# KMASAHIRO/AVR

Hardware: AMD Instinct MI355X
Metric: ray-samples/sec/GPU (1024 rays×256 samp×512 freq) + IR render ms/pose (higher is better)
Workload: dtype f32; 1 GPU; c2_meshrir_1024x256x512; mode=pose, rays=1024, samples=256, T=1022, freq_bins=512, distinct_poses=16, parallelism=poses x1 (no data-path collective)

## Files before the change

avr_amd/_lib.py:

```python
from __future__ import annotations

import ctypes
import math
import os
import threading

import numpy as np

_HERE = os.path.dirname(os.path.abspath(__file__))
LIB_PATH = os.path.join(_HERE, "libavr_hip.so")

DTYPE_F32 = 0
DTYPE_F16 = 1
DTYPE_BF16 = 2
MAX_AZI = 512

_c_i32 = ctypes.c_int32
_c_i64 = ctypes.c_int64
_c_f32 = ctypes.c_float
_vp = ctypes.c_void_p


class RenderParams(ctypes.Structure):

# ... 35 lines not shown
    p.n_samples = int(cfg["n_samples"])
    p.T = int(T)
    p.n_rays = p.n_azi * p.n_ele + 2 if n_rays is None else int(n_rays)
    p.depth_scale = _f32(cfg["far"] - cfg["near"])
    p.depth_offset = _f32(cfg["near"])
    p.lo = _f32(cfg["xyz_min"])
    p.span = _f32(cfg["xyz_max"] - cfg["xyz_min"])
    p.fs = _f32(cfg["fs"])
    p.speed = _f32(cfg["speed"])
    p.pathloss = _f32(cfg["pathloss"])
    p.azi_jitter = _f32(np.pi * 2 / cfg["n_azi"])
    p.two_pi = _f32(np.pi * 2)
    p.phase_c = _f32((-2 * np.pi) / T)
    p.near_clamp = int(0.1 / cfg["speed"] * cfg["fs"])
    p.pl_len = int(math.ceil(T * 2.5))
    return p


class TablePtrs(ctypes.Structure):

    _fields_ = [("d_vals", ctypes.c_void_p), ("shift", ctypes.c_void_p),
                ("pl_table", ctypes.c_void_p), ("phase", ctypes.c_void_p),
                ("twiddle", ctypes.c_void_p), ("ir_twiddle", ctypes.c_void_p)]


_SIGS = {
    "avr_last_error": (ctypes.c_char_p, []),
    "avr_abi_version": (ctypes.c_int, []),
    "avr_pinned_alloc": (ctypes.c_int, [_c_i64, _vp, _vp]),
    "avr_pinned_free": (ctypes.c_int, [_vp]),
    "avr_graph_launch": (ctypes.c_int, [_vp, _vp]),
    "avr_tables": (ctypes.c_int, [_vp, _vp, _vp, _vp, _vp, _vp, _vp, _vp]),
    "avr_depth_samples": (ctypes.c_int, [_vp, _vp, _vp]),
    "avr_ir_twiddle": (ctypes.c_int, [_c_i32, _vp, _vp]),
    "avr_ray_directions": (ctypes.c_int, [_vp, _vp, _vp, _vp]),
    "avr_sample_points": (ctypes.c_int, [_vp, _c_i32] + [_vp] * 10),
    "avr_sample_rays": (ctypes.c_int, [_vp, _c_i32, _vp, _c_i32] + [_vp] * 9),
    "avr_weights_fwd": (ctypes.c_int, [_vp, _c_i32, _vp, _c_i32] + [_vp] * 7),
    "avr_ray_reduce_fwd": (ctypes.c_int, [_vp, _c_i32, _vp, _c_i32, _vp, _vp, _c_i32, _vp, _vp]),
    "avr_sample_rays_dev": (ctypes.c_int, [_vp, _c_i32, _vp, _c_i32] + [_vp] * 9),
    "avr_sample_rays_staged": (ctypes.c_int, [_vp, _c_i32, _vp, _c_i32, _c_i32] + [_vp] * 7),
    "avr_reduce_splits": (ctypes.c_int, [_vp, _c_i32, _c_i32, _vp]),
    "avr_dft_phase_fwd": (ctypes.c_int, [_vp, _c_i32, _vp, _c_i32, _vp, _vp, _vp, _vp, _c_i32, _vp, _vp]),
    "avr_spectrum_finalize": (ctypes.c_int, [_c_i32, _c_i32, _c_i32, _vp, _vp, _vp]),
    "avr_irfft": (ctypes.c_int, [_c_i32, _c_i32, _vp, _vp, _vp, _vp]),
    "avr_irfft_bwd": (ctypes.c_int, [_c_i32, _c_i32, _vp, _vp, _vp, _vp]),
# ... 35 lines not shown
    "avr_head_bwd2": (ctypes.c_int, [_vp, _c_i32, _c_i32, _vp, _vp, _c_i32, _vp, _vp, _vp, _vp, _vp, _vp,
                                     _c_i32, _vp, _vp, _vp, _vp, _c_i64, _vp]),
    "avr_criterion_window_len": (ctypes.c_int, []),
    "avr_criterion_workspace": (ctypes.c_int, [_c_i32, _c_i32, _vp]),
    "avr_criterion_fwd": (ctypes.c_int, [_c_i32, _c_i32] + [_vp] * 10 + [_c_i64, _vp]),
    "avr_criterion_fwd2": (ctypes.c_int, [_c_i32, _c_i32] + [_vp] * 11 + [_c_i64, _vp]),
    "avr_criterion_bwd": (ctypes.c_int, [_c_i32, _c_i32] + [_vp] * 11 + [_c_i64, _vp, _vp]),
    "avr_das_workspace": (ctypes.c_int, [_vp]),
    "avr_das_fwd": (ctypes.c_int, [_c_i32] + [_vp] * 5 + [_c_f32] * 3 + [_vp, _vp, _c_i64, _vp]),
    "avr_das_bwd": (ctypes.c_int, [_c_i32] + [_vp] * 3 + [_c_f32] * 3 + [_vp, _vp, _c_i64, _vp, _vp]),
    "avr_scale_sanitize": (ctypes.c_int, [_c_i32, _vp, _vp, _vp, _vp]),
    "avr_grad_clip_workspace": (ctypes.c_int, [_c_i32, _vp, _vp]),
    "avr_grad_clip_coef": (ctypes.c_int, [_c_i32, _vp, _vp, ctypes.c_float, _vp, ctypes.c_int64, _vp, _vp, _vp]),
    "avr_adam_step": (ctypes.c_int, [_c_i32, _vp, _vp, _vp, _vp, _vp, _vp, _vp, ctypes.c_double, ctypes.c_double,
                                     ctypes.c_float, ctypes.c_float, _vp, _vp]),
    "avr_concat_fwd": (ctypes.c_int, [_c_i64, _c_i32, _vp, _vp, _c_i32, _vp]),
    "avr_concat_bwd": (ctypes.c_int, [_c_i64, _c_i32, _vp, _vp, _c_i32, _vp, _vp]),
    "avr_sigma_pack_bytes": (ctypes.c_int, [_c_i32, _vp]),
    "avr_sigma_desc_size": (ctypes.c_int, []),
    "avr_sigma_fwd": (ctypes.c_int, [_vp] * 3 + [_c_i32, _vp, _vp]),
    "avr_render_core_layout": (ctypes.c_int, [_vp, _c_i32, _c_i32, _vp, _vp]),
    "avr_render_core_fwd": (ctypes.c_int, [_vp, _c_i32, _vp, _c_i32, _vp, _c_i32] + [_vp] * 5
                            + [_c_i64] + [_vp] * 5),
}

EXPORTS = tuple(_SIGS)

_SHAPES_SIGS = {
    "avr_linear512_pack_w": (ctypes.c_int, [_vp, _c_i32, _vp, _vp]),
    "avr_linear512_relu_fwd": (ctypes.c_int, [_c_i64, _vp, _vp, _c_i32, _vp, _vp]),
    "avr_mlp512x2_pack_w": (ctypes.c_int, [_vp, _vp, _c_i32, _vp, _vp]),
    "avr_mlp512x2_fwd": (ctypes.c_int, [_c_i64, _vp, _vp, _c_i32, _vp, _vp]),
    "avr_linear_pack_w": (ctypes.c_int, [_c_i32, _c_i32, _vp, _c_i32, _vp, _vp]),
}

_lock = threading.Lock()
_lib = None


def load():
    global _lib
    if _lib is not None:
        return _lib
    with _lock:
        if _lib is not None:
            return _lib
# ... 27 lines not shown
```

avr_amd/csrc/common.h:

```cpp
#pragma once

#include <hip/hip_runtime.h>
#include <hip/hip_fp16.h>
#include <hip/hip_bf16.h>
#include <type_traits>
#include <stdint.h>
#include <string>

#include "avr_hip.h"

namespace avr {

void set_error(const std::string& msg);
int fail(int code, const std::string& msg);
int check_launch(const char* what);
int device_cus();

#define AVR_REQUIRE(cond, msg)                          \
    do {                                                \
        if (!(cond)) return ::avr::fail(AVR_E_ARG, msg); \
    } while (0)

int launch_irfft(int B, int F, const float* spec, const float* spec2, const float* tw, float* ir,
                 float* ir2, void* stream);

inline hipStream_t as_stream(void* s) { return reinterpret_cast<hipStream_t>(s); }

__device__ __forceinline__ void mfma_queue_wait() {
    __builtin_amdgcn_sched_barrier(0);
    asm volatile("s_nop 7");
}
template <typename T>
__device__ __forceinline__ void keep_live(const T& v) {
    asm volatile("" ::"v"(v));
}

__device__ __forceinline__ float load_f(const float* p, int64_t i) { return p[i]; }
__device__ __forceinline__ float load_f(const __half* p, int64_t i) { return __half2float(p[i]); }
__device__ __forceinline__ float load_f(const __hip_bfloat16* p, int64_t i) {
    return __bfloat162float(p[i]);
}
__device__ __forceinline__ void store_f(float* p, int64_t i, float v) { p[i] = v; }
__device__ __forceinline__ void store_f(__half* p, int64_t i, float v) { p[i] = __float2half(v); }
__device__ __forceinline__ void store_f(__hip_bfloat16* p, int64_t i, float v) {
    p[i] = __float2bfloat16(v);
}
__device__ __forceinline__ float bf16_lo(uint32_t u) { return __uint_as_float(u << 16); }
// ... 174 lines not shown
```

avr_amd/csrc/render_fwd.hip:

```cpp
#include "common.h"

#include <cstdlib>

using namespace avr;

typedef float floatx16 __attribute__((ext_vector_type(16)));

namespace {

constexpr double kTwoPi = 6.283185307179586476925286766559;

__global__ void tables_kernel(avr_render_params p, float* __restrict__ d_vals,
                              float* __restrict__ frac, int32_t* __restrict__ shift,
                              float* __restrict__ pl, float2* __restrict__ phase,
                              float2* __restrict__ tw) {
    const int S = p.n_samples, T = p.T, F = T / 2 + 1;
    const int64_t gid = (int64_t)blockIdx.x * blockDim.x + threadIdx.x;
    const int64_t stride = (int64_t)gridDim.x * blockDim.x;
    for (int64_t i = gid; i < S; i += stride) {
        const float d = linspace_at(0.0f, 1.0f, S, (int)i) * p.depth_scale + p.depth_offset;
        const float fr = (p.fs * d) / p.speed;
        d_vals[i] = d;
        frac[i] = fr;
        shift[i] = (int32_t)rintf(fr);
// ... 1019 lines not shown
    avr_reduce_splits(p, B, sig_dtype, &ns);
    L.n_split = ns;
    const int nkc = (int)((T + kKc - 1) / kKc);
    int ks = 1;
    if (const char* f = getenv("AVR_KSPLIT")) {
        ks = atoi(f);
    } else {
        const int64_t base = ((F + 127) / 128) * ((S + 31) / 32) * B;
        ks = (int)((256 + (base > 0 ? base : 1) - 1) / (base > 0 ? base : 1));
    }
    if (ks < 1) ks = 1;
    if (ks > nkc) ks = nkc;
    L.k_split = ks;
    L.P = (int32_t)(((S + 31) / 32) * ks);
    auto al = [](int64_t x) { return (x + 255) & ~(int64_t)255; };
    int64_t o = 0;
    L.w = o;
    o += al((int64_t)B * R * S * 4);
    L.delay = o;
    o += al((int64_t)B * R * S * 4);
    L.part = o;
    o += al((int64_t)ns * B * S * T * 4);
    L.spart = o;
    o += al((int64_t)B * L.P * F * 8);
    L.bytes = o;
    return L;
}
}

extern "C" int avr_render_core_layout(const avr_render_params* p, int32_t B, int32_t sig_dtype,
                                      int64_t* offsets ,
                                      int32_t* splits ) {
    if (int e = validate(p)) return e;
    AVR_REQUIRE(B >= 1 && offsets && splits, "avr_render_core_layout: bad args");
    const CoreLayout L = core_layout(p, B, sig_dtype);
    offsets[0] = L.w;
    offsets[1] = L.delay;
    offsets[2] = L.part;
    offsets[3] = L.spart;
    offsets[4] = L.bytes;
    splits[0] = L.n_split;
    splits[1] = L.k_split;
    return 0;
}

extern "C" int avr_render_core_fwd(const avr_render_params* p, int32_t B, const void* attn,
                                   int32_t attn_dtype, const void* signal, int32_t sig_dtype,
                                   const float* rays_o, const float* pos_tx, const float* dirs,
                                   const avr_table_ptrs* tab, void* workspace,
                                   int64_t workspace_bytes, float* out, float* ir, void* ev_begin,
                                   void* ev_end, void* stream) {
    if (int e = validate(p)) return e;
    AVR_REQUIRE(tab && workspace && out, "avr_render_core_fwd: null pointer");
    const CoreLayout L = core_layout(p, B, sig_dtype);
    AVR_REQUIRE(workspace_bytes >= L.bytes, "avr_render_core_fwd: workspace too small");
    char* ws = reinterpret_cast<char*>(workspace);
    float* w = reinterpret_cast<float*>(ws + L.w);
    int32_t* delay = reinterpret_cast<int32_t*>(ws + L.delay);
    float* part = reinterpret_cast<float*>(ws + L.part);
    float* spart = reinterpret_cast<float*>(ws + L.spart);
    if (int e = avr_weights_fwd(p, B, attn, attn_dtype, rays_o, pos_tx, dirs, tab->d_vals, w, delay, stream))
        return e;
    hipStream_t s = as_stream(stream);
    if (ev_begin) (void)hipEventRecord(reinterpret_cast<hipEvent_t>(ev_begin), s);
    if (int e = avr_ray_reduce_fwd(p, B, signal, sig_dtype, w, delay, L.n_split, part, stream))
        return e;
    if (ev_end) (void)hipEventRecord(reinterpret_cast<hipEvent_t>(ev_end), s);
    if (int e = avr_dft_phase_fwd(p, B, part, L.n_split, tab->pl_table, tab->shift, tab->phase, tab->twiddle,
                                  L.k_split, spart, stream))
        return e;
    if (int e = avr_spectrum_finalize(B, L.P, p->T / 2 + 1, spart, out, stream)) return e;
    if (ir) {
        AVR_REQUIRE(tab->ir_twiddle, "avr_render_core_fwd: ir requested without ir_twiddle");
        return avr_irfft(B, p->T / 2 + 1, out, tab->ir_twiddle, ir, stream);
    }
    return 0;
}
```

avr_amd/renderer.py:

```python
from __future__ import annotations

import ctypes
import math
import threading

import torch
import torch.nn as nn

from . import _lib
from ._lib import DTYPE_BF16, DTYPE_F16, DTYPE_F32, render_params
from .options import tuning_env
from .wcache import cache_lookup, cache_store, capturing, cast_weight


_RENDER_KEYS = ("n_samples", "near", "far", "n_azi", "n_ele", "speed", "fs", "pathloss",
                "xyz_min", "xyz_max")


def _ptr(t):
    return None if t is None else t.data_ptr()


def _stream(device):
    return torch.cuda.current_stream(device).cuda_stream
# ... 38 lines not shown
        f32 = dict(dtype=torch.float32, device=device)
        self.d_vals = torch.empty(S, **f32)
        self.frac = torch.empty(S, **f32)
        self.shift = torch.empty(S, dtype=torch.int32, device=device)
        self.pl = torch.empty(p.pl_len, **f32)
        self.phase = torch.empty(S, F, 2, **f32)
        self.twiddle = torch.empty(T, 2, **f32)
        n = 2 * (F - 1)
        self.ir_n = n
        self.ir_twiddle = torch.empty(max(n, 2), 2, **f32)
        st = _stream(device)
        with torch.cuda.device(device):
            _lib.call("avr_tables", ctypes_ref(p), _ptr(self.d_vals), _ptr(self.frac),
                      _ptr(self.shift), _ptr(self.pl), _ptr(self.phase), _ptr(self.twiddle), st)
            if n >= 2:
                _lib.call("avr_ir_twiddle", n, _ptr(self.ir_twiddle), st)
        shifts = self.shift.cpu()
        self.max_shift = int(shifts.max().item()) if S > 0 else 0
        self.ptrs = _lib.TablePtrs(self.d_vals.data_ptr(), self.shift.data_ptr(),
                                   self.pl.data_ptr(), self.phase.data_ptr(),
                                   self.twiddle.data_ptr(),
                                   self.ir_twiddle.data_ptr() if n >= 2 else None)
        self._layouts = {}

    def core_layout(self, p, B, sig_code):
        key = (p.n_rays, B, sig_code) + tuning_env()
        v = self._layouts.get(key)
        if v is None:
            with _TABLE_LOCK:
                v = self._layouts.get(key)
                if v is None:
                    off = (ctypes.c_int64 * 5)()
                    sp = (ctypes.c_int32 * 2)()
                    _lib.call("avr_render_core_layout", ctypes_ref(p), B, sig_code, off, sp)
                    v = (tuple(off), int(sp[0]), int(sp[1]))
                    self._layouts[key] = v
        return v


def ctypes_ref(p):
    import ctypes

    return ctypes.byref(p)


_TABLE_CACHE: dict = {}
# ... 33 lines not shown

def pick_k_split(B, S, T):
    F = T // 2 + 1
    nkc = math.ceil(T / 64)
    forced = tuning_env()[1]
    forced = int(forced) if forced else None
    if forced:
        return max(1, min(nkc, forced))
    base = math.ceil(F / 128) * math.ceil(S / 32) * B
    return max(1, min(nkc, math.ceil(256 / max(1, base))))


def _weights(p, attn, rays_o, position_tx, dirs, tables, st):
    B = attn.size(0)
    R, S = p.n_rays, p.n_samples
    dev = attn.device
    w = torch.empty(B, R, S, dtype=torch.float32, device=dev)
    delay = torch.empty(B, R, S, dtype=torch.int32, device=dev)
    _lib.call("avr_weights_fwd", ctypes_ref(p), B, _ptr(attn), _dtype_code(attn), _ptr(rays_o),
              _ptr(position_tx), _ptr(dirs), _ptr(tables.d_vals), _ptr(w), _ptr(delay), st)
    return w, delay


def _spectrum(p, tables, part, n_split, B, dev, st):
    S, T = p.n_samples, p.T
    F = T // 2 + 1
    k_split = pick_k_split(B, S, T)
    P = math.ceil(S / 32) * k_split
    spart = torch.empty(B, P, F, 2, dtype=torch.float32, device=dev)
    _lib.call("avr_dft_phase_fwd", ctypes_ref(p), B, _ptr(part), n_split, _ptr(tables.pl),
              _ptr(tables.shift), _ptr(tables.phase), _ptr(tables.twiddle), k_split,
              _ptr(spart), st)
    out = torch.empty(B, F, 2, dtype=torch.float32, device=dev)
    _lib.call("avr_spectrum_finalize", B, P, F, _ptr(spart), _ptr(out), st)
    return out


def _grad_z(p, tables, grad_out, B, dev, st):
    g = grad_out.contiguous().float()
    gz = torch.empty(B, p.n_samples, p.T, dtype=torch.float32, device=dev)
    _lib.call("avr_dft_phase_bwd", ctypes_ref(p), B, _ptr(g), _ptr(tables.pl), _ptr(tables.shift),
              _ptr(tables.phase), _ptr(tables.twiddle), _ptr(gz), st)
    return gz


def _grad_attn(p, tables, attn, grad_w, st):
    grad_attn = torch.empty_like(attn)
    _lib.call("avr_weights_bwd", ctypes_ref(p), attn.size(0), _ptr(attn), _dtype_code(attn),
              _ptr(tables.d_vals), _ptr(grad_w), _ptr(grad_attn), st)
    return grad_attn


def _render_core_fwd(attn, signal, p, tables, rays_o, position_tx, dirs, ir_out, timer=None):
    dev = signal.device
    B = signal.size(0)
    F = p.T // 2 + 1
    sig_code = _dtype_code(signal)
    off, n_split, _ = tables.core_layout(p, B, sig_code)
    ws = torch.empty(off[4], dtype=torch.uint8, device=dev)
    out = torch.empty(B, F, 2, dtype=torch.float32, device=dev)
    ev0 = ev1 = None
    if timer is not None:
        R, S = p.n_rays, p.n_samples
        delay = ws[off[1]:off[1] + B * R * S * 4].view(torch.int32).view(B, R, S)
        ev0, ev1 = timer.events(n_split=n_split, delay=delay, shift=tables.shift)
    _lib.call("avr_render_core_fwd", ctypes_ref(p), B, _ptr(attn), _dtype_code(attn),
              _ptr(signal), sig_code, _ptr(rays_o), _ptr(position_tx), _ptr(dirs),
              ctypes.byref(tables.ptrs), _ptr(ws), off[4], _ptr(out), _ptr(ir_out), ev0, ev1,
              _stream(dev))
    return out, ws, off


class RenderCore(torch.autograd.Function):

    @staticmethod
    def forward(ctx, attn, signal, p, tables, rays_o, position_tx, dirs, ir_out=None, timer=None):
        out, ws, off = _render_core_fwd(attn, signal, p, tables, rays_o, position_tx, dirs, ir_out, timer)
        B, R, S = signal.size(0), p.n_rays, p.n_samples
        w = ws[off[0]:off[0] + B * R * S * 4].view(torch.float32).view(B, R, S)
        delay = ws[off[1]:off[1] + B * R * S * 4].view(torch.int32).view(B, R, S)
        ctx.p, ctx.tables = p, tables
        ctx.save_for_backward(attn, signal, w, delay)
        return out

    @staticmethod
    def backward(ctx, grad_out):
        attn, signal, w, delay = ctx.saved_tensors
        p, tables = ctx.p, ctx.tables
        dev = signal.device
        B = signal.size(0)
        R, S = p.n_rays, p.n_samples
        st = _stream(dev)
        gz = _grad_z(p, tables, grad_out, B, dev, st)
        grad_signal = torch.empty_like(signal)
        grad_w = torch.empty(B, R, S, dtype=torch.float32, device=dev)
        _lib.call("avr_ray_reduce_bwd", ctypes_ref(p), B, _ptr(signal), _dtype_code(signal),
                  _ptr(gz), _ptr(w), _ptr(delay), _ptr(grad_signal), _ptr(grad_w), st)
        grad_attn = _grad_attn(p, tables, attn, grad_w, st) if ctx.needs_input_grad[0] else None
        return (grad_attn, grad_signal if ctx.needs_input_grad[1] else None,
                None, None, None, None, None, None, None)


def _packed_head_weight(w_master, W, cache, pref, shape_key, st):
    key = (W.data_ptr(), w_master._version, shape_key)
    cache = cache and not capturing()
    if cache:
        hit = cache_lookup(w_master, "_avr_headpack", key)
        if hit is not None:
            return hit
    B, K, code = shape_key[2], shape_key[3], shape_key[4]
    Wp = torch.empty_like(W)
    _lib.call("avr_head_pack_w", pref, B, K, _ptr(W), code, _ptr(Wp), st)
    return cache_store(w_master, "_avr_headpack", key, Wp) if cache else Wp


def _packed_exact_weight(w_master, W, cache, pref, shape_key, nbytes, st):
    key = (W.data_ptr(), w_master._version, shape_key)
    cache = cache and not capturing()
    if cache:
        hit = cache_lookup(w_master, "_avr_exactpack", key)
        if hit is not None:
            return hit
    K, code = shape_key[1], shape_key[2]
    Wf = torch.empty(nbytes // 2, dtype=W.dtype, device=W.device)
    _lib.call("avr_head_pack_w_exact", pref, K, _ptr(W), code, _ptr(Wf), st)
    return cache_store(w_master, "_avr_exactpack", key, Wf) if cache else Wf


class FusedHeadCore(torch.autograd.Function):

    @staticmethod
    def forward(ctx, attn, h, w_master, dtype, p, tables, rays_o, position_tx, dirs, cache=False, exact=False,
                relu_h=False, timer=None):
        dev = h.device
        B, K = h.size(0), h.size(-1)
        S, T = p.n_samples, p.T
        st = _stream(dev)
        pref = ctypes_ref(p)
        W = cast_weight(w_master, dtype, cache)
        code = _dtype_code(h)
        w, delay = _weights(p, attn, rays_o, position_tx, dirs, tables, st)
        R = p.n_rays
        perm = torch.empty(B, S, R, dtype=torch.int32, device=dev)
        ws = torch.empty(B, S, R, dtype=torch.float32, device=dev)
        cnt = torch.empty(B, S, T, dtype=torch.int32, device=dev)
        _lib.call("avr_head_sort", pref, B, _ptr(w), _ptr(delay), _ptr(perm), _ptr(ws), _ptr(cnt), st)
        if exact:
            ns, wbytes = ctypes.c_int32(0), ctypes.c_int64(0)
            _lib.call("avr_head_exact_layout", pref, B, K, code, ctypes.byref(ns), ctypes.byref(wbytes))
            n_split = ns.value
            part = torch.empty(n_split, B, S, T, dtype=torch.float32, device=dev)
            queue = torch.empty(256, dtype=torch.int32, device=dev)
            Wf = _packed_exact_weight(w_master, W, cache, pref, (p.T, K, code), wbytes.value, st)
            ev0, ev1 = timer.head_events(delay, tables.shift, K) if timer is not None else (None, None)
            if ev0 is not None:
                ev0.record()
            _lib.call("avr_head_fwd_exact", pref, B, K, _ptr(h), _ptr(Wf), code, _ptr(perm), _ptr(ws), _ptr(cnt),
                      _ptr(delay), n_split, _ptr(part), _ptr(queue), st)
            if ev1 is not None:
                ev1.record()
        else:
            ns = ctypes.c_int32(0)
            _lib.call("avr_head_splits", pref, B, K, code, ctypes.byref(ns))
            n_split = ns.value
            part = torch.empty(n_split, B, S, T, dtype=torch.float32, device=dev)
            Wp = _packed_head_weight(w_master, W, cache, pref, (p.T, R, B, K, code), st)
            _lib.call("avr_head_fwd", pref, B, K, _ptr(h), _ptr(Wp), code, _ptr(perm), _ptr(ws), _ptr(cnt),
                      n_split, _ptr(part), st)
        out = _spectrum(p, tables, part, n_split, B, dev, st)
        ctx.p, ctx.tables, ctx.relu_h = p, tables, relu_h
        ctx.save_for_backward(attn, h, W, w, delay, perm, ws, cnt)
        return out

    @staticmethod
    def backward(ctx, grad_out):
        attn, h, W, w, delay, perm, ws, cnt = ctx.saved_tensors
        p, tables = ctx.p, ctx.tables
        dev = h.device
        B, K = h.size(0), h.size(-1)
        R, S, T = p.n_rays, p.n_samples, p.T
        st = _stream(dev)
        pref = ctypes_ref(p)
        code = _dtype_code(h)
        gz = _grad_z(p, tables, grad_out, B, dev, st)
        nbytes = ctypes.c_int64(0)
        _lib.call("avr_head_bwd_workspace", pref, B, K, code, ctypes.byref(nbytes))
        work = torch.empty(max(1, nbytes.value // 4), dtype=torch.float32, device=dev)
        grad_h = torch.empty_like(h)
        grad_w = torch.empty(B, R, S, dtype=torch.float32, device=dev)
        grad_W = torch.empty(T, K, dtype=torch.float32, device=dev)
        _lib.call("avr_head_bwd2", pref, B, K, _ptr(h), _ptr(W), code, _ptr(w), _ptr(delay), _ptr(perm),
                  _ptr(ws), _ptr(cnt), _ptr(gz), int(ctx.relu_h), _ptr(grad_h), _ptr(grad_w), _ptr(grad_W),
                  _ptr(work), nbytes.value, st)
        grad_attn = _grad_attn(p, tables, attn, grad_w, st) if ctx.needs_input_grad[0] else None
        return (grad_attn, grad_h if ctx.needs_input_grad[1] else None,
                grad_W if ctx.needs_input_grad[2] else None, None, None, None, None, None, None, None, None, None,
                None)


def _poison_nonfinite(out, tensors, ir_out=None):
    bad = None
    for t in tensors:
        b = ~torch.isfinite(t).all()
        bad = b if bad is None else bad | b
    poison = torch.where(bad, float("nan"), 0.0)
    if ir_out is not None:
        ir_out.add_(poison)
    return out + poison


def normalize_points(input_pts, xyz_min, xyz_max):
    return 2 * (input_pts - xyz_min) / (xyz_max - xyz_min) - 1


def denormalize_points(input_pts, xyz_min, xyz_max):
    return (input_pts + 1) / 2 * (xyz_max - xyz_min) + xyz_min


def draw_jitter(n_azi, n_ele):
    u_azi = torch.rand(n_azi)
# ... 7 lines not shown
    if not random_azi:
        u = torch.zeros_like(u)
    p = render_params(dict(n_azi=n_azi, n_ele=n_ele, n_samples=1, far=1, near=0, xyz_min=-1,
                           xyz_max=1, fs=1, speed=1, pathloss=1), 2)
    dirs = torch.empty(n_azi * n_ele + 2, 3, dtype=torch.float32, device=device)
    u_dev = u.to(device, non_blocking=True)
    _lib.call("avr_ray_directions", ctypes_ref(p), _ptr(u_dev), _ptr(dirs), _stream(device))
    return dirs, None, None


class AVRRender(nn.Module):

    def __init__(self, networks_fn, **kwargs) -> None:
        super().__init__()
        self.network_fn = networks_fn
        for k in _RENDER_KEYS:
            setattr(self, k, kwargs[k])
        self._cfg = {k: kwargs[k] for k in _RENDER_KEYS}
        self.ray_range = None
        self.fused_head = bool(kwargs.get("fused_head", True))
        self.propagate_nonfinite = bool(kwargs.get("propagate_nonfinite", False))
        self.exact_head = bool(kwargs.get("exact_head", True))
        self.head_relu_link = bool(kwargs.get("head_relu_link", True))
        self._pcache = {}
        self._pcache_lock = threading.Lock()
        self._jitter_dev = None
        self._staged = None
        self.kernel_timer = None

    def _device(self, rays_o):
        if rays_o.is_cuda:
            return rays_o.device
        if not torch.cuda.is_available():
            raise RuntimeError("avr_amd.AVRRender needs a HIP device (no CPU fallback)")
        return torch.device("cuda", torch.cuda.current_device())

    def sample(self, rays_o, position_tx, direction_tx=None, u_azi=None):
        if self._staged is not None:
            return self._sample_staged(position_tx.size(0), direction_tx is not None)
        dev = self._device(rays_o)
        B = position_tx.size(0)
        u_dev = self._jitter_dev if u_azi is None else None
        if u_azi is not None and u_azi.is_cuda:
            u_dev, u_azi = u_azi.to(dev, torch.float32).contiguous(), None
        if u_azi is None and u_dev is None:
            u_azi = draw_jitter(self.n_azi, self.n_ele)
# ... 83 lines not shown
        if signal.dtype not in native:
            signal = signal.float()
        if attn.device != dev:
            attn = attn.to(dev)
        attn = attn.reshape(B, -1)
        if not attn.is_contiguous():
            attn = attn.contiguous()
        T = signal.size(-1)
        if signal.device != dev:
            signal = signal.to(dev)
        signal = signal.reshape(B, -1, T)
        if not signal.is_contiguous():
            signal = signal.contiguous()
        R = geom["n_rays"]
        if attn.size(1) != R * S or signal.size(1) != R * S:
            raise ValueError(f"network output has {signal.size(1)} ray-samples, expected "
                             f"{R}x{S}={R * S}")
        p = self._params(T, R)
        with _on(dev):
            tables = get_tables(p, dev)
            check_config(p, tables)
            if not (torch.is_grad_enabled() and (attn.requires_grad or signal.requires_grad)):
                out = _render_core_fwd(attn, signal, p, tables, geom["rays_o"],
                                       geom["position_tx"], geom["dirs"], ir_out, self.kernel_timer)[0]
            else:
                out = RenderCore.apply(attn, signal, p, tables, geom["rays_o"], geom["position_tx"],
                                       geom["dirs"], ir_out, self.kernel_timer)
            if self.propagate_nonfinite:
                out = _poison_nonfinite(out, (attn, signal), ir_out)
            return out

    def _head_supported(self, geom, h, weight, dtype):
        if dtype not in (torch.float32, torch.bfloat16, torch.float16):
            return False
        p = self._params(weight.size(0), geom["n_rays"])
        code = {torch.bfloat16: DTYPE_BF16, torch.float16: DTYPE_F16}.get(dtype, DTYPE_F32)
        n = ctypes.c_int32(0)
        lib = _lib.load()
        if lib.avr_head_splits(ctypes_ref(p), geom["B"], h.size(-1), code, ctypes.byref(n)) != 0:
            return False
        if self._exact_for(dtype, h.size(-1)):
            nb = ctypes.c_int64(0)
            return lib.avr_head_exact_layout(ctypes_ref(p), geom["B"], h.size(-1), code, ctypes.byref(n),
                                             ctypes.byref(nb)) == 0
        return True

    def _exact_for(self, dtype, K):
        return self.exact_head and dtype in (torch.float16, torch.bfloat16) and K % 16 == 0 and K <= 512

    def render_from_hidden(self, attn, h, weight, dtype, geom, relu_link=None):
        dev, B = geom["device"], geom["B"]
        S = int(self.n_samples)
        attn = attn.to(dev).reshape(B, -1)
        if attn.dtype not in (torch.float32, torch.float16, torch.bfloat16):
            attn = attn.float()
        attn = attn.contiguous()
        K, T = h.size(-1), weight.size(0)
        h = h.to(dev, dtype).reshape(B, -1, K).contiguous()
        R = geom["n_rays"]
        if attn.size(1) != R * S or h.size(1) != R * S:
            raise ValueError(f"network output has {h.size(1)} ray-samples, expected {R}x{S}={R * S}")
        p = self._params(T, R)
        with _on(dev):
            tables = get_tables(p, dev)
            check_config(p, tables)
            exact = self._exact_for(dtype, K)
            relu_h = relu_link is not None and torch.is_grad_enabled()
            out = FusedHeadCore.apply(attn, h, weight, dtype, p, tables, geom["rays_o"],
                                      geom["position_tx"], geom["dirs"], not torch.is_grad_enabled(), exact,
                                      relu_h, self.kernel_timer)
            if relu_h:
                relu_link[0] = True
            if self.propagate_nonfinite:
                out = _poison_nonfinite(out, (attn, h, weight))
            return out

    def forward(self, rays_o, position_tx, direction_tx=None, ch_idx=None):
        return self._render(rays_o, position_tx, direction_tx, ch_idx, None)

    def render_ir(self, rays_o, position_tx, direction_tx=None, ch_idx=None):
        ir = []
        grad = torch.is_grad_enabled()
        out = self._render(rays_o, position_tx, direction_tx, ch_idx, None if grad else ir)
        return out, (ir[0] if ir else spectrum_to_ir(out))

    def _render(self, rays_o, position_tx, direction_tx, ch_idx, ir_slot, u_azi=None):
        pts, view, tx, dtx, geom = self.sample(rays_o, position_tx, direction_tx, u_azi=u_azi)
        kw = {} if ch_idx is None else {"ch_idx": ch_idx}
        if getattr(self.network_fn, "accepts_ray_layout", False):
            kw["ray_layout"] = (geom["B"], geom["n_rays"], int(self.n_samples))
        net_in = (pts, view, tx) if dtx is None else (pts, view, tx, dtx)
        if self.fused_head and getattr(self.network_fn, "supports_fused_head", False):
            attn, h, weight, dtype = self.network_fn.forward_fused(*net_in, **kw)
# ... 70 lines not shown
```

include/avr_hip.h:

```cpp
#ifndef AVR_HIP_H
#define AVR_HIP_H

#include <stdint.h>

#ifdef __cplusplus
extern "C" {
#endif

#define AVR_ABI_VERSION 2

#define AVR_DTYPE_F32 0
#define AVR_DTYPE_F16 1
#define AVR_DTYPE_BF16 2

#define AVR_E_ARG 1001
#define AVR_E_CONFIG 1002

typedef struct avr_render_params {
    int32_t n_azi;
    int32_t n_ele;
    int32_t n_samples;
    int32_t T;
    int32_t n_rays;
    float depth_scale;
// ... 67 lines not shown

int avr_irfft(int32_t B, int32_t F, const float* spec, const float* tw, float* ir,
              void* stream);
int avr_irfft_bwd(int32_t B, int32_t F, const float* grad_ir, const float* tw, float* grad_spec,
                  void* stream);

typedef struct avr_table_ptrs {
    const float* d_vals;
    const int32_t* shift;
    const float* pl_table;
    const float* phase;
    const float* twiddle;
    const float* ir_twiddle;
} avr_table_ptrs;

int avr_render_core_layout(const avr_render_params* p, int32_t B, int32_t sig_dtype,
                           int64_t* offsets, int32_t* splits);

int avr_render_core_fwd(const avr_render_params* p, int32_t B, const void* attn,
                        int32_t attn_dtype, const void* signal, int32_t sig_dtype,
                        const float* rays_o, const float* pos_tx, const float* dirs,
                        const avr_table_ptrs* tables, void* workspace, int64_t workspace_bytes,
                        float* out, float* ir, void* ev_begin, void* ev_end, void* stream);

int avr_dft_phase_bwd(const avr_render_params* p, int32_t B, const float* grad_out,
                      const float* pl_table, const int32_t* shift, const float* phase,
                      const float* twiddle, float* gz, void* stream);

int avr_ray_reduce_bwd(const avr_render_params* p, int32_t B, const void* signal,
                       int32_t sig_dtype, const float* gz, const float* w,
                       const int32_t* delay, void* grad_signal, float* grad_w, void* stream);

int avr_weights_bwd(const avr_render_params* p, int32_t B, const void* attn, int32_t attn_dtype,
                    const float* d_vals, const float* grad_w, void* grad_attn, void* stream);

int avr_hashgrid_fwd(int64_t N, int32_t n_levels, const float* x, const void* params,
                     int32_t param_dtype, const int64_t* level_offset, const float* level_scale,
                     const int32_t* level_res, void* out, int32_t out_dtype, void* stream);

int avr_hashgrid_fwd_lm(int64_t N, int32_t n_levels, const float* x, const void* params,
                        int32_t param_dtype, const int64_t* level_offset, const float* level_scale,
                        const int32_t* level_res, void* out, int32_t out_dtype, void* stream);
int avr_hashgrid_fwd_lm_unit(int64_t N, int32_t n_levels, const float* x, const void* params,
                             int32_t param_dtype, const int64_t* level_offset, const float* level_scale,
                             const int32_t* level_res, void* out, int32_t out_dtype, void* stream);

// ... 156 lines not shown
```

Before: 2.298 billion ray-samples/s.

## Replace dense per-sample DFT with Bluestein FFT in the forward spectrum

Adds a Bluestein chirp-z FFT kernel that runs in LDS and computes the per-sample spectrum (T=1022, padded to a power of two). It processes two real samples per complex transform, then applies the per-sample phase and accumulates per frequency. This replaces the dense O(T·F) DFT with O(N log N) work per sample and is selected automatically when T>=254. The cost is precomputed host tables, new workspace sizing, and some loss of f32 accuracy from the chirp-based transform.

```diff
diff --git a/avr_amd/_lib.py b/avr_amd/_lib.py
--- a/avr_amd/_lib.py
+++ b/avr_amd/_lib.py
@@ -81,6 +81,11 @@
     _fields_ = [("d_vals", ctypes.c_void_p), ("shift", ctypes.c_void_p),
                 ("pl_table", ctypes.c_void_p), ("phase", ctypes.c_void_p),
                 ("twiddle", ctypes.c_void_p), ("ir_twiddle", ctypes.c_void_p)]
+
+
+class FftPtrs(ctypes.Structure):
+
+    _fields_ = [("chirp", ctypes.c_void_p), ("filter", ctypes.c_void_p), ("twiddle", ctypes.c_void_p)]
 
 
 _SIGS = {
@@ -162,6 +167,12 @@
     "avr_render_core_layout": (ctypes.c_int, [_vp, _c_i32, _c_i32, _vp, _vp]),
     "avr_render_core_fwd": (ctypes.c_int, [_vp, _c_i32, _vp, _c_i32, _vp, _c_i32] + [_vp] * 5
                             + [_c_i64] + [_vp] * 5),
+    "avr_render_core_fwd_dft": (ctypes.c_int, [_vp, _c_i32, _vp, _c_i32, _vp, _c_i32] + [_vp] * 6
+                                + [_c_i64] + [_vp] * 5),
+    "avr_fft_size": (ctypes.c_int, [_c_i32, _vp]),
+    "avr_fft_tables": (ctypes.c_int, [_vp] * 5),
+    "avr_dft_fft_layout": (ctypes.c_int, [_vp, _c_i32, _vp, _vp]),
+    "avr_dft_fft_fwd": (ctypes.c_int, [_vp, _c_i32, _vp, _c_i32, _vp, _vp, _vp, _vp, _c_i32, _vp, _vp]),
 }
 
 EXPORTS = tuple(_SIGS)
diff --git a/avr_amd/csrc/common.h b/avr_amd/csrc/common.h
--- a/avr_amd/csrc/common.h
+++ b/avr_amd/csrc/common.h
@@ -23,6 +23,9 @@
 
 int launch_irfft(int B, int F, const float* spec, const float* spec2, const float* tw, float* ir,
                  float* ir2, void* stream);
+
+bool fft_preferred(int B, int S, int T);
+int fft_slots(int B, int S, int T);
 
 inline hipStream_t as_stream(void* s) { return reinterpret_cast<hipStream_t>(s); }
 
diff --git a/avr_amd/csrc/fft.hip b/avr_amd/csrc/fft.hip
--- /dev/null
+++ b/avr_amd/csrc/fft.hip
@@ -0,0 +1,359 @@
+#include "common.h"
+
+#include <cmath>
+#include <complex>
+#include <vector>
+
+using namespace avr;
+
+namespace {
+
+constexpr double kPi = 3.14159265358979323846264338327950288;
+constexpr int kFftMaxN = 8192;
+constexpr int kFftMaxThreads = 512;
+
+__host__ __device__ inline int fft_len(int T) {
+    int n = 4;
+    while (n < 2 * T - 1) n *= 2;
+    return n;
+}
+inline int ilog2(int n) {
+    int l = 0;
+    while ((1 << l) < n) ++l;
+    return l;
+}
+
+__device__ __forceinline__ float2 cmul(float2 a, float2 b) {
+    return make_float2(a.x * b.x - a.y * b.y, a.x * b.y + a.y * b.x);
+}
+__device__ __forceinline__ float2 cmulc(float2 a, float2 b) {
+    return make_float2(a.x * b.x + a.y * b.y, a.y * b.x - a.x * b.y);
+}
+__device__ __forceinline__ float2 cadd(float2 a, float2 b) { return make_float2(a.x + b.x, a.y + b.y); }
+__device__ __forceinline__ float2 csub(float2 a, float2 b) { return make_float2(a.x - b.x, a.y - b.y); }
+
+__device__ __forceinline__ void bfly4_fwd(float2& a0, float2& a1, float2& a2, float2& a3) {
+    const float2 t0 = cadd(a0, a2), t1 = csub(a0, a2), t2 = cadd(a1, a3), d = csub(a1, a3);
+    const float2 t3 = make_float2(d.y, -d.x);
+    a0 = cadd(t0, t2);
+    a1 = cadd(t1, t3);
+    a2 = csub(t0, t2);
+    a3 = csub(t1, t3);
+}
+__device__ __forceinline__ void bfly4_inv(float2& a0, float2& a1, float2& a2, float2& a3) {
+    const float2 t0 = cadd(a0, a2), t1 = csub(a0, a2), t2 = cadd(a1, a3), d = csub(a1, a3);
+    const float2 t3 = make_float2(-d.y, d.x);
+    a0 = cadd(t0, t2);
+    a1 = cadd(t1, t3);
+    a2 = csub(t0, t2);
+    a3 = csub(t1, t3);
+}
+
+template <bool INV>
+__device__ __forceinline__ void radix4_stage(float2* __restrict__ x, const float2* __restrict__ tw,
+                                             int N, int lq) {
+    const int q = 1 << lq;
+    for (int i = threadIdx.x; i < (N >> 2); i += blockDim.x) {
+        const int j = i & (q - 1);
+        const int base = ((i >> lq) << (lq + 2)) + j;
+        float2 a0 = x[base], a1 = x[base + q], a2 = x[base + 2 * q], a3 = x[base + 3 * q];
+        const float2 w1 = tw[j], w2 = tw[q + j], w3 = tw[2 * q + j];
+        if (INV) {
+            a1 = cmulc(a1, w1);
+            a2 = cmulc(a2, w2);
+            a3 = cmulc(a3, w3);
+            bfly4_inv(a0, a1, a2, a3);
+        } else {
+            bfly4_fwd(a0, a1, a2, a3);
+            a1 = cmul(a1, w1);
+            a2 = cmul(a2, w2);
+            a3 = cmul(a3, w3);
+        }
+        x[base] = a0;
+        x[base + q] = a1;
+        x[base + 2 * q] = a2;
+        x[base + 3 * q] = a3;
+    }
+}
+
+template <int NS>
+__global__ __launch_bounds__(kFftMaxThreads) void dft_fft_fwd_kernel(
+    const float* __restrict__ part, const float* __restrict__ pl, const int32_t* __restrict__ shift,
+    const float2* __restrict__ phase, const float2* __restrict__ chirp,
+    const float2* __restrict__ filt, const float2* __restrict__ twg, float2* __restrict__ spart,
+    int B, int S, int T, int N, int logN, int G, int P) {
+    extern __shared__ float2 lds[];
+    float2* x = lds;
+    float2* tw = lds + N;
+    const int F = T / 2 + 1;
+    const int b = blockIdx.y, p = blockIdx.x;
+    const int tid = threadIdx.x, nt = blockDim.x;
+    const bool odd = logN & 1;
+    const int logN2 = odd ? logN - 1 : logN;
+    const int64_t slab = (int64_t)B * S * T;
+    const int npairs = (S + 1) >> 1;
+
+    const int qmax = 1 << (logN2 - 2);
+    const float2* roots2 = tw + (N >> 1);
+    for (int i = tid; i < N; i += nt) tw[i] = twg[i];
+
+    constexpr int kAcc = 5;
+    float2 acc[kAcc];
+#pragma unroll
+    for (int k = 0; k < kAcc; ++k) acc[k] = make_float2(0.0f, 0.0f);
+
+    for (int g = 0; g < G; ++g) {
+        const int pair = p * G + g;
+        if (pair >= npairs) break;
+        const int s0 = 2 * pair, s1 = s0 + 1;
+        const bool has1 = s1 < S;
+        const int sh0 = shift[s0], sh1 = has1 ? shift[s1] : 0;
+        const int lim0 = T - 1 - sh0, lim1 = has1 ? T - 1 - sh1 : 0;
+        const float* r0 = part + ((int64_t)b * S + s0) * T;
+        const float* r1 = part + ((int64_t)b * S + (has1 ? s1 : s0)) * T;
+        __syncthreads();
+        const int half = N >> 1;
+        for (int t = tid; t < (odd ? half : N); t += nt) {
+            float2 a = make_float2(0.0f, 0.0f);
+            if (t < T) {
+                float z0 = 0.0f, z1 = 0.0f;
+                if (t < lim0) {
+                    float sum = r0[t];
+#pragma unroll
+                    for (int k = 1; k < NS; ++k) sum += r0[k * slab + t];
+                    z0 = sum * pl[sh0 + t];
+                }
+                if (t < lim1) {
+                    float sum = r1[t];
+#pragma unroll
+                    for (int k = 1; k < NS; ++k) sum += r1[k * slab + t];
+                    z1 = sum * pl[sh1 + t];
+                }
+                const float2 c = chirp[t];
+                a = make_float2(z0 * c.x - z1 * c.y, z0 * c.y + z1 * c.x);
+            }
+            x[t] = a;
+            if (odd) x[t + half] = (t < T) ? cmul(a, roots2[t]) : a;
+        }
+        __syncthreads();
+        for (int lq = logN2 - 2; lq >= 2; lq -= 2) {
+            radix4_stage<false>(x, tw + 4 * (qmax - (1 << lq)), N, lq);
+            __syncthreads();
+        }
+        for (int i = tid; i < (N >> 2); i += nt) {
+            float4* xv = reinterpret_cast<float4*>(x + 4 * i);
+            const float4* fv = reinterpret_cast<const float4*>(filt + 4 * i);
+            const float4 u = xv[0], v = xv[1], fu = fv[0], fw = fv[1];
+            float2 a0 = make_float2(u.x, u.y), a1 = make_float2(u.z, u.w);
+            float2 a2 = make_float2(v.x, v.y), a3 = make_float2(v.z, v.w);
+            bfly4_fwd(a0, a1, a2, a3);
+            a0 = cmul(a0, make_float2(fu.x, fu.y));
+            a1 = cmul(a1, make_float2(fu.z, fu.w));
+            a2 = cmul(a2, make_float2(fw.x, fw.y));
+            a3 = cmul(a3, make_float2(fw.z, fw.w));
+            bfly4_inv(a0, a1, a2, a3);
+            xv[0] = make_float4(a0.x, a0.y, a1.x, a1.y);
+            xv[1] = make_float4(a2.x, a2.y, a3.x, a3.y);
+        }
+        __syncthreads();
+        for (int lq = 2; lq <= logN2 - 2; lq += 2) {
+            radix4_stage<true>(x, tw + 4 * (qmax - (1 << lq)), N, lq);
+            __syncthreads();
+        }
+        auto X = [&](int f) {
+            float2 y = x[f];
+            if (odd) y = cadd(y, cmulc(x[f + half], roots2[f]));
+            return cmul(y, chirp[f]);
+        };
+#pragma unroll
+        for (int k = 0; k < kAcc; ++k) {
+            const int f = tid + k * nt;
+            if (f < F) {
+                const float2 xa = X(f);
+                const float2 xb = X(f == 0 ? 0 : T - f);
+                const float2 z0 = make_float2(0.5f * (xa.x + xb.x), 0.5f * (xa.y - xb.y));
+                const float2 d = make_float2(xa.x - xb.x, xa.y + xb.y);
+                const float2 z1 = make_float2(0.5f * d.y, -0.5f * d.x);
+                const float2 q0 = cmul(z0, phase[(int64_t)s0 * F + f]);
+                acc[k] = cadd(acc[k], q0);
+                if (has1) {
+                    const float2 q1 = cmul(z1, phase[(int64_t)s1 * F + f]);
+                    acc[k] = cadd(acc[k], q1);
+                }
+            }
+        }
+    }
+#pragma unroll
+    for (int k = 0; k < kAcc; ++k) {
+        const int f = tid + k * nt;
+        if (f < F) spart[((int64_t)b * P + p) * F + f] = acc[k];
+    }
+}
+
+
+struct FftShape {
+    int N, logN, G, P, threads;
+};
+FftShape fft_shape(int B, int S, int T) {
+    FftShape sh{};
+    sh.N = fft_len(T);
+    sh.logN = ilog2(sh.N);
+    const int npairs = (S + 1) / 2;
+    const int64_t total = (int64_t)npairs * B;
+    sh.G = (int)((total + 255) / 256);
+    sh.P = (npairs + sh.G - 1) / sh.G;
+    sh.threads = sh.N / 4 < 64 ? 64 : (sh.N / 4 > kFftMaxThreads ? kFftMaxThreads : sh.N / 4);
+    return sh;
+}
+
+bool fft_params_ok(const avr_render_params* p) {
+    return p && p->T >= 2 && p->T <= 16384 && p->n_samples >= 1 && p->n_samples <= 8192;
+}
+
+void host_dif(std::vector<std::complex<double>>& x, const std::vector<std::complex<double>>& w) {
+    using cd = std::complex<double>;
+    const int N = (int)x.size(), logN = ilog2(N);
+    int len = N;
+    if (logN & 1) {
+        const int h = N / 2;
+        for (int j = 0; j < h; ++j) {
+            const cd a = x[j], b = x[j + h];
+            x[j] = a + b;
+            x[j + h] = (a - b) * w[j];
+        }
+        len = h;
+    }
+    const cd mi(0.0, -1.0);
+    for (int L = len; L >= 4; L /= 4) {
+        const int q = L / 4, step = N / L;
+        for (int base0 = 0; base0 < N; base0 += L)
+            for (int j = 0; j < q; ++j) {
+                cd* e = &x[base0 + j];
+                const cd a0 = e[0], a1 = e[q], a2 = e[2 * q], a3 = e[3 * q];
+                const cd t0 = a0 + a2, t1 = a0 - a2, t2 = a1 + a3, t3 = (a1 - a3) * mi;
+                e[0] = t0 + t2;
+                e[q] = (t1 + t3) * w[j * step];
+                e[2 * q] = (t0 - t2) * w[2 * j * step];
+                e[3 * q] = (t1 - t3) * w[3 * j * step];
+            }
+    }
+}
+
+}
+
+extern "C" int avr_fft_size(int32_t T, int32_t* N) {
+    AVR_REQUIRE(T >= 2 && T <= 16384 && N, "avr_fft_size: bad args");
+    *N = fft_len(T);
+    return 0;
+}
+
+extern "C" int avr_fft_tables(const avr_render_params* p, float* chirp, float* filt, float* twiddle,
+                              void* stream) {
+    AVR_REQUIRE(fft_params_ok(p) && chirp && filt && twiddle, "avr_fft_tables: bad args");
+    using cd = std::complex<double>;
+    const int T = p->T, N = fft_len(T);
+    std::vector<cd> w(N), c(T), b(N, cd(0.0, 0.0));
+    for (int k = 0; k < N; ++k) {
+        const double a = 2.0 * kPi * (double)k / (double)N;
+        w[k] = cd(std::cos(a), -std::sin(a));
+    }
+    for (int n = 0; n < T; ++n) {
+        const int64_t m = ((int64_t)n * n) % (2 * (int64_t)T);
+        const double a = kPi * (double)m / (double)T;
+        c[n] = cd(std::cos(a), -std::sin(a));
+    }
+    for (int n = 0; n < T; ++n) {
+        b[n] = std::conj(c[n]);
+        if (n) b[N - n] = std::conj(c[n]);
+    }
+    host_dif(b, w);
+    std::vector<cd> tw(N, cd(0.0, 0.0));
+    {
+        const int logN = ilog2(N), odd = logN & 1, logN2 = logN - odd;
+        const int qmax = 1 << (logN2 - 2);
+        for (int lq = logN2 - 2; lq >= 2; lq -= 2) {
+            const int q = 1 << lq, step = N / (4 * q);
+            cd* t = &tw[4 * (size_t)(qmax - q)];
+            for (int k = 1; k <= 3; ++k)
+                for (int j = 0; j < q; ++j) t[(size_t)(k - 1) * q + j] = w[(size_t)j * k * step];
+        }
+        if (odd)
+            for (int j = 0; j < N / 2; ++j) tw[N / 2 + j] = w[j];
+    }
+    std::vector<float> hc(2 * (size_t)T), hf(2 * (size_t)N), hw(2 * (size_t)N);
+    for (int n = 0; n < T; ++n) {
+        hc[2 * n] = (float)c[n].real();
+        hc[2 * n + 1] = (float)c[n].imag();
+    }
+    for (int k = 0; k < N; ++k) {
+        hf[2 * k] = (float)(b[k].real() / (double)N);
+        hf[2 * k + 1] = (float)(b[k].imag() / (double)N);
+        hw[2 * k] = (float)tw[k].real();
+        hw[2 * k + 1] = (float)tw[k].imag();
+    }
+    hipStream_t s = as_stream(stream);
+    hipError_t e = hipMemcpyAsync(chirp, hc.data(), hc.size() * sizeof(float), hipMemcpyHostToDevice, s);
+    if (e == hipSuccess) e = hipMemcpyAsync(filt, hf.data(), hf.size() * sizeof(float), hipMemcpyHostToDevice, s);
+    if (e == hipSuccess) e = hipMemcpyAsync(twiddle, hw.data(), hw.size() * sizeof(float), hipMemcpyHostToDevice, s);
+    if (e == hipSuccess) e = hipStreamSynchronize(s);
+    if (e != hipSuccess) return fail((int)e, std::string("avr_fft_tables: ") + hipGetErrorString(e));
+    return 0;
+}
+
+extern "C" int avr_dft_fft_layout(const avr_render_params* p, int32_t B, int32_t* P, int32_t* prefer) {
+    AVR_REQUIRE(fft_params_ok(p) && B >= 1 && P && prefer, "avr_dft_fft_layout: bad args");
+    const FftShape sh = fft_shape(B, p->n_samples, p->T);
+    if (sh.N > kFftMaxN) {
+        *P = 0;
+        *prefer = 0;
+        return 0;
+    }
+    *P = sh.P;
+    *prefer = avr::fft_preferred(B, p->n_samples, p->T) ? 1 : 0;
+    return 0;
+}
+
+extern "C" int avr_dft_fft_fwd(const avr_render_params* p, int32_t B, const float* part, int32_t n_split,
+                               const float* pl_table, const int32_t* shift, const float* phase,
+                               const avr_fft_ptrs* fft, int32_t P, float* spart, void* stream) {
+    AVR_REQUIRE(fft_params_ok(p) && B >= 1 && part && pl_table && shift && phase && fft && fft->chirp &&
+                    fft->filter && fft->twiddle && spart,
+                "avr_dft_fft_fwd: bad args");
+    const int S = p->n_samples, T = p->T;
+    const FftShape sh = fft_shape(B, S, T);
+    AVR_REQUIRE(sh.N <= kFftMaxN, "avr_dft_fft_fwd: T too large for the LDS transform (N > 8192)");
+    AVR_REQUIRE(P == sh.P, "avr_dft_fft_fwd: P does not match avr_dft_fft_layout");
+    const size_t lds = (size_t)sh.N * 2 * sizeof(float2);
+    auto go = [&](auto kern) {
+        if (lds > 65536)
+            (void)hipFuncSetAttribute((const void*)kern, hipFuncAttributeMaxDynamicSharedMemorySize,
+                                      (int)lds);
+        hipLaunchKernelGGL(kern, dim3((unsigned)sh.P, (unsigned)B), dim3(sh.threads), lds, as_stream(stream),
+                           part, pl_table, shift, reinterpret_cast<const float2*>(phase),
+                           reinterpret_cast<const float2*>(fft->chirp),
+                           reinterpret_cast<const float2*>(fft->filter),
+                           reinterpret_cast<const float2*>(fft->twiddle), reinterpret_cast<float2*>(spart),
+                           (int)B, S, T, sh.N, sh.logN, sh.G, sh.P);
+    };
+    switch (n_split) {
+        case 1: go(dft_fft_fwd_kernel<1>); break;
+        case 2: go(dft_fft_fwd_kernel<2>); break;
+        case 4: go(dft_fft_fwd_kernel<4>); break;
+        case 8: go(dft_fft_fwd_kernel<8>); break;
+        case 16: go(dft_fft_fwd_kernel<16>); break;
+        default: return fail(AVR_E_ARG, "avr_dft_fft_fwd: n_split must be 1, 2, 4, 8 or 16");
+    }
+    return check_launch("avr_dft_fft_fwd");
+}
+
+namespace avr {
+bool fft_preferred(int B, int S, int T) {
+    (void)B;
+    (void)S;
+    return fft_len(T) <= kFftMaxN && T >= 254;
+}
+int fft_slots(int B, int S, int T) {
+    const FftShape sh = fft_shape(B, S, T);
+    return sh.N <= kFftMaxN ? sh.P : 0;
+}
+}
diff --git a/avr_amd/csrc/render_fwd.hip b/avr_amd/csrc/render_fwd.hip
--- a/avr_amd/csrc/render_fwd.hip
+++ b/avr_amd/csrc/render_fwd.hip
@@ -1065,7 +1065,8 @@
     L.part = o;
     o += al((int64_t)ns * B * S * T * 4);
     L.spart = o;
-    o += al((int64_t)B * L.P * F * 8);
+    const int64_t pf = fft_slots(B, (int)S, (int)T);
+    o += al((int64_t)B * (pf > L.P ? pf : L.P) * F * 8);
     L.bytes = o;
     return L;
 }
@@ -1087,12 +1088,12 @@
     return 0;
 }
 
-extern "C" int avr_render_core_fwd(const avr_render_params* p, int32_t B, const void* attn,
-                                   int32_t attn_dtype, const void* signal, int32_t sig_dtype,
-                                   const float* rays_o, const float* pos_tx, const float* dirs,
-                                   const avr_table_ptrs* tab, void* workspace,
-                                   int64_t workspace_bytes, float* out, float* ir, void* ev_begin,
-                                   void* ev_end, void* stream) {
+extern "C" int avr_render_core_fwd_dft(const avr_render_params* p, int32_t B, const void* attn,
+                                       int32_t attn_dtype, const void* signal, int32_t sig_dtype,
+                                       const float* rays_o, const float* pos_tx, const float* dirs,
+                                       const avr_table_ptrs* tab, const avr_fft_ptrs* fft,
+                                       void* workspace, int64_t workspace_bytes, float* out, float* ir,
+                                       void* ev_begin, void* ev_end, void* stream) {
     if (int e = validate(p)) return e;
     AVR_REQUIRE(tab && workspace && out, "avr_render_core_fwd: null pointer");
     const CoreLayout L = core_layout(p, B, sig_dtype);
@@ -1109,13 +1110,30 @@
     if (int e = avr_ray_reduce_fwd(p, B, signal, sig_dtype, w, delay, L.n_split, part, stream))
         return e;
     if (ev_end) (void)hipEventRecord(reinterpret_cast<hipEvent_t>(ev_end), s);
-    if (int e = avr_dft_phase_fwd(p, B, part, L.n_split, tab->pl_table, tab->shift, tab->phase, tab->twiddle,
-                                  L.k_split, spart, stream))
+    int P = L.P;
+    if (fft) {
+        P = fft_slots(B, p->n_samples, p->T);
+        if (int e = avr_dft_fft_fwd(p, B, part, L.n_split, tab->pl_table, tab->shift, tab->phase, fft, P, spart,
+                                    stream))
+            return e;
+    } else if (int e = avr_dft_phase_fwd(p, B, part, L.n_split, tab->pl_table, tab->shift, tab->phase,
+                                         tab->twiddle, L.k_split, spart, stream)) {
         return e;
-    if (int e = avr_spectrum_finalize(B, L.P, p->T / 2 + 1, spart, out, stream)) return e;
+    }
+    if (int e = avr_spectrum_finalize(B, P, p->T / 2 + 1, spart, out, stream)) return e;
     if (ir) {
         AVR_REQUIRE(tab->ir_twiddle, "avr_render_core_fwd: ir requested without ir_twiddle");
         return avr_irfft(B, p->T / 2 + 1, out, tab->ir_twiddle, ir, stream);
     }
     return 0;
 }
+
+extern "C" int avr_render_core_fwd(const avr_render_params* p, int32_t B, const void* attn,
+                                   int32_t attn_dtype, const void* signal, int32_t sig_dtype,
+                                   const float* rays_o, const float* pos_tx, const float* dirs,
+                                   const avr_table_ptrs* tab, void* workspace,
+                                   int64_t workspace_bytes, float* out, float* ir, void* ev_begin,
+                                   void* ev_end, void* stream) {
+    return avr_render_core_fwd_dft(p, B, attn, attn_dtype, signal, sig_dtype, rays_o, pos_tx, dirs, tab,
+                                   nullptr, workspace, workspace_bytes, out, ir, ev_begin, ev_end, stream);
+}
diff --git a/avr_amd/renderer.py b/avr_amd/renderer.py
--- a/avr_amd/renderer.py
+++ b/avr_amd/renderer.py
@@ -84,6 +84,41 @@
                                    self.twiddle.data_ptr(),
                                    self.ir_twiddle.data_ptr() if n >= 2 else None)
         self._layouts = {}
+        P, prefer = ctypes.c_int32(0), ctypes.c_int32(0)
+        _lib.call("avr_dft_fft_layout", ctypes_ref(p), 1, ctypes.byref(P), ctypes.byref(prefer))
+        self.fft = None
+        self._fft_layouts = {}
+        if P.value > 0:
+            n_fft = ctypes.c_int32(0)
+            _lib.call("avr_fft_size", T, ctypes.byref(n_fft))
+            self.fft_n = n_fft.value
+            self.chirp = torch.empty(T, 2, **f32)
+            self.fft_filter = torch.empty(self.fft_n, 2, **f32)
+            self.fft_twiddle = torch.empty(self.fft_n, 2, **f32)
+            with torch.cuda.device(device):
+                _lib.call("avr_fft_tables", ctypes_ref(p), _ptr(self.chirp), _ptr(self.fft_filter),
+                          _ptr(self.fft_twiddle), st)
+            self.fft = _lib.FftPtrs(self.chirp.data_ptr(), self.fft_filter.data_ptr(),
+                                    self.fft_twiddle.data_ptr())
+
+    def fft_layout(self, p, B):
+        v = self._fft_layouts.get(B)
+        if v is None:
+            P, prefer = ctypes.c_int32(0), ctypes.c_int32(0)
+            _lib.call("avr_dft_fft_layout", ctypes_ref(p), B, ctypes.byref(P), ctypes.byref(prefer))
+            v = (P.value, bool(prefer.value))
+            self._fft_layouts[B] = v
+        return v
+
+    def use_fft(self, p, B, dft):
+        if dft == "dense":
+            return False
+        P, prefer = self.fft_layout(p, B) if self.fft is not None else (0, False)
+        if dft == "fft":
+            if P <= 0:
+                raise RuntimeError(f"dft='fft': T={p.T} needs a transform longer than 8192 (dense only)")
+            return True
+        return prefer
 
     def core_layout(self, p, B, sig_code):
         key = (p.n_rays, B, sig_code) + tuning_env()
@@ -163,15 +198,21 @@
     return w, delay
 
 
-def _spectrum(p, tables, part, n_split, B, dev, st):
+def dft_fwd(p, tables, part, n_split, B, dev, st, dft="auto"):
     S, T = p.n_samples, p.T
     F = T // 2 + 1
-    k_split = pick_k_split(B, S, T)
-    P = math.ceil(S / 32) * k_split
-    spart = torch.empty(B, P, F, 2, dtype=torch.float32, device=dev)
-    _lib.call("avr_dft_phase_fwd", ctypes_ref(p), B, _ptr(part), n_split, _ptr(tables.pl),
-              _ptr(tables.shift), _ptr(tables.phase), _ptr(tables.twiddle), k_split,
-              _ptr(spart), st)
+    if tables.use_fft(p, B, dft):
+        P = tables.fft_layout(p, B)[0]
+        spart = torch.empty(B, P, F, 2, dtype=torch.float32, device=dev)
+        _lib.call("avr_dft_fft_fwd", ctypes_ref(p), B, _ptr(part), n_split, _ptr(tables.pl),
+                  _ptr(tables.shift), _ptr(tables.phase), ctypes.byref(tables.fft), P, _ptr(spart), st)
+    else:
+        k_split = pick_k_split(B, S, T)
+        P = math.ceil(S / 32) * k_split
+        spart = torch.empty(B, P, F, 2, dtype=torch.float32, device=dev)
+        _lib.call("avr_dft_phase_fwd", ctypes_ref(p), B, _ptr(part), n_split, _ptr(tables.pl),
+                  _ptr(tables.shift), _ptr(tables.phase), _ptr(tables.twiddle), k_split,
+                  _ptr(spart), st)
     out = torch.empty(B, F, 2, dtype=torch.float32, device=dev)
     _lib.call("avr_spectrum_finalize", B, P, F, _ptr(spart), _ptr(out), st)
     return out
@@ -192,7 +233,7 @@
     return grad_attn
 
 
-def _render_core_fwd(attn, signal, p, tables, rays_o, position_tx, dirs, ir_out, timer=None):
+def _render_core_fwd(attn, signal, p, tables, rays_o, position_tx, dirs, ir_out, timer=None, dft="auto"):
     dev = signal.device
     B = signal.size(0)
     F = p.T // 2 + 1
@@ -205,9 +246,10 @@
         R, S = p.n_rays, p.n_samples
         delay = ws[off[1]:off[1] + B * R * S * 4].view(torch.int32).view(B, R, S)
         ev0, ev1 = timer.events(n_split=n_split, delay=delay, shift=tables.shift)
-    _lib.call("avr_render_core_fwd", ctypes_ref(p), B, _ptr(attn), _dtype_code(attn),
+    fft = ctypes.byref(tables.fft) if tables.use_fft(p, B, dft) else None
+    _lib.call("avr_render_core_fwd_dft", ctypes_ref(p), B, _ptr(attn), _dtype_code(attn),
               _ptr(signal), sig_code, _ptr(rays_o), _ptr(position_tx), _ptr(dirs),
-              ctypes.byref(tables.ptrs), _ptr(ws), off[4], _ptr(out), _ptr(ir_out), ev0, ev1,
+              ctypes.byref(tables.ptrs), fft, _ptr(ws), off[4], _ptr(out), _ptr(ir_out), ev0, ev1,
               _stream(dev))
     return out, ws, off
 
@@ -215,8 +257,9 @@
 class RenderCore(torch.autograd.Function):
 
     @staticmethod
-    def forward(ctx, attn, signal, p, tables, rays_o, position_tx, dirs, ir_out=None, timer=None):
-        out, ws, off = _render_core_fwd(attn, signal, p, tables, rays_o, position_tx, dirs, ir_out, timer)
+    def forward(ctx, attn, signal, p, tables, rays_o, position_tx, dirs, ir_out=None, timer=None, dft="auto"):
+        out, ws, off = _render_core_fwd(attn, signal, p, tables, rays_o, position_tx, dirs, ir_out, timer,
+                                        dft)
         B, R, S = signal.size(0), p.n_rays, p.n_samples
         w = ws[off[0]:off[0] + B * R * S * 4].view(torch.float32).view(B, R, S)
         delay = ws[off[1]:off[1] + B * R * S * 4].view(torch.int32).view(B, R, S)
@@ -239,7 +282,7 @@
                   _ptr(gz), _ptr(w), _ptr(delay), _ptr(grad_signal), _ptr(grad_w), st)
         grad_attn = _grad_attn(p, tables, attn, grad_w, st) if ctx.needs_input_grad[0] else None
         return (grad_attn, grad_signal if ctx.needs_input_grad[1] else None,
-                None, None, None, None, None, None, None)
+                None, None, None, None, None, None, None, None)
 
 
 def _packed_head_weight(w_master, W, cache, pref, shape_key, st):
@@ -272,7 +315,7 @@
 
     @staticmethod
     def forward(ctx, attn, h, w_master, dtype, p, tables, rays_o, position_tx, dirs, cache=False, exact=False,
-                relu_h=False, timer=None):
+                relu_h=False, timer=None, dft="auto"):
         dev = h.device
         B, K = h.size(0), h.size(-1)
         S, T = p.n_samples, p.T
@@ -308,7 +351,7 @@
             Wp = _packed_head_weight(w_master, W, cache, pref, (p.T, R, B, K, code), st)
             _lib.call("avr_head_fwd", pref, B, K, _ptr(h), _ptr(Wp), code, _ptr(perm), _ptr(ws), _ptr(cnt),
                       n_split, _ptr(part), st)
-        out = _spectrum(p, tables, part, n_split, B, dev, st)
+        out = dft_fwd(p, tables, part, n_split, B, dev, st, dft)
         ctx.p, ctx.tables, ctx.relu_h = p, tables, relu_h
         ctx.save_for_backward(attn, h, W, w, delay, perm, ws, cnt)
         return out
@@ -336,7 +379,7 @@
         grad_attn = _grad_attn(p, tables, attn, grad_w, st) if ctx.needs_input_grad[0] else None
         return (grad_attn, grad_h if ctx.needs_input_grad[1] else None,
                 grad_W if ctx.needs_input_grad[2] else None, None, None, None, None, None, None, None, None, None,
-                None)
+                None, None)
 
 
 def _poison_nonfinite(out, tensors, ir_out=None):
@@ -390,6 +433,9 @@
         self.propagate_nonfinite = bool(kwargs.get("propagate_nonfinite", False))
         self.exact_head = bool(kwargs.get("exact_head", True))
         self.head_relu_link = bool(kwargs.get("head_relu_link", True))
+        self.dft = str(kwargs.get("dft", "auto"))
+        if self.dft not in ("auto", "fft", "dense"):
+            raise ValueError(f"dft must be 'auto', 'fft' or 'dense', got {self.dft!r}")
         self._pcache = {}
         self._pcache_lock = threading.Lock()
         self._jitter_dev = None
@@ -519,10 +565,11 @@
             check_config(p, tables)
             if not (torch.is_grad_enabled() and (attn.requires_grad or signal.requires_grad)):
                 out = _render_core_fwd(attn, signal, p, tables, geom["rays_o"],
-                                       geom["position_tx"], geom["dirs"], ir_out, self.kernel_timer)[0]
+                                       geom["position_tx"], geom["dirs"], ir_out, self.kernel_timer,
+                                       self.dft)[0]
             else:
                 out = RenderCore.apply(attn, signal, p, tables, geom["rays_o"], geom["position_tx"],
-                                       geom["dirs"], ir_out, self.kernel_timer)
+                                       geom["dirs"], ir_out, self.kernel_timer, self.dft)
             if self.propagate_nonfinite:
                 out = _poison_nonfinite(out, (attn, signal), ir_out)
             return out
@@ -565,7 +612,7 @@
             relu_h = relu_link is not None and torch.is_grad_enabled()
             out = FusedHeadCore.apply(attn, h, weight, dtype, p, tables, geom["rays_o"],
                                       geom["position_tx"], geom["dirs"], not torch.is_grad_enabled(), exact,
-                                      relu_h, self.kernel_timer)
+                                      relu_h, self.kernel_timer, self.dft)
             if relu_h:
                 relu_link[0] = True
             if self.propagate_nonfinite:
diff --git a/include/avr_hip.h b/include/avr_hip.h
--- a/include/avr_hip.h
+++ b/include/avr_hip.h
@@ -113,6 +113,25 @@
                         const float* rays_o, const float* pos_tx, const float* dirs,
                         const avr_table_ptrs* tables, void* workspace, int64_t workspace_bytes,
                         float* out, float* ir, void* ev_begin, void* ev_end, void* stream);
+
+typedef struct avr_fft_ptrs {
+    const float* chirp;
+    const float* filter;
+    const float* twiddle;
+} avr_fft_ptrs;
+int avr_fft_size(int32_t T, int32_t* N);
+int avr_fft_tables(const avr_render_params* p, float* chirp, float* filter, float* twiddle,
+                   void* stream);
+int avr_dft_fft_layout(const avr_render_params* p, int32_t B, int32_t* P, int32_t* prefer);
+int avr_dft_fft_fwd(const avr_render_params* p, int32_t B, const float* part, int32_t n_split,
+                    const float* pl_table, const int32_t* shift, const float* phase,
+                    const avr_fft_ptrs* fft, int32_t P, float* spart, void* stream);
+int avr_render_core_fwd_dft(const avr_render_params* p, int32_t B, const void* attn,
+                            int32_t attn_dtype, const void* signal, int32_t sig_dtype,
+                            const float* rays_o, const float* pos_tx, const float* dirs,
+                            const avr_table_ptrs* tables, const avr_fft_ptrs* fft, void* workspace,
+                            int64_t workspace_bytes, float* out, float* ir, void* ev_begin,
+                            void* ev_end, void* stream);
 
 int avr_dft_phase_bwd(const avr_render_params* p, int32_t B, const float* grad_out,
                       const float* pl_table, const int32_t* shift, const float* phase,
```

Measured after the change: 2.314 billion ray-samples/s, median of 6. About the same (+0.7%).
